# Paleogenomics/pss-bam

Hardware: AMD Instinct MI355X
Metric: aligned reads/s (whole node) + HBM GB/s fraction, 200M x 150bp BAM (higher is better)
Workload: dtype u64

## Files before the change

pss-bam_amd/csrc/bgzf_api.h:

```cpp
#pragma once

#include "inflate_kernels.h"
#include "inflate_wave.h"

extern "C" int64_t pssbam_bgzf_scan(const void *bytes, uint64_t nbytes, pssbam_bgzf_block *blocks, uint64_t max_blocks,
                                    uint64_t *consumed, uint64_t *inflated_bytes) {
    const uint8_t *p = (const uint8_t *)bytes;
    uint64_t o = 0, n = 0, uoff = 0;
    while (o + 18 <= nbytes && (!blocks || n < max_blocks)) {
        if (p[o] != 0x1f || p[o + 1] != 0x8b || p[o + 2] != 8 || !(p[o + 3] & 4)) { fail(PSSBAM_EFORMAT, "not a BGZF block at offset %llu", (unsigned long long)o); return PSSBAM_EFORMAT; }
        const uint32_t xlen = p[o + 10] | ((uint32_t)p[o + 11] << 8);
        if (o + 12 + xlen > nbytes) break;
        uint32_t bsize = 0;
        bool found = false;
        for (uint32_t x = 0; x + 4 <= xlen;) {
            const uint8_t *sf = p + o + 12 + x;
            const uint32_t slen = sf[2] | ((uint32_t)sf[3] << 8);
            if (sf[0] == 'B' && sf[1] == 'C' && slen == 2 && x + 6 <= xlen) { bsize = (sf[4] | ((uint32_t)sf[5] << 8)) + 1u; found = true; break; }
            x += 4 + slen;
        }
        if (!found || bsize < 12u + xlen + 8u) { fail(PSSBAM_EFORMAT, "BGZF block at offset %llu has no usable BC field", (unsigned long long)o); return PSSBAM_EFORMAT; }
        if (o + bsize > nbytes) break;
        uint32_t crc, isize;
        memcpy(&crc, p + o + bsize - 8, 4);
// ... 557 lines not shown
    (void)hipGetLastError();
    size_t limit = FEED_SLOTS_READY;
    if (const char *v = getenv("PSSBAM_FEED_SLOTS")) limit = std::max<size_t>(2, (size_t)atoi(v));
    if (!feed_engine_ready(e)) {
        if (!e->feed_mem_budget) {
            size_t free_b = 0, total_b = 0;
            if (hipMemGetInfo(&free_b, &total_b) != hipSuccess) free_b = 64ull << 30;
            const uint64_t used = e->feed.size() * feed_slot_bytes(e);
            const uint64_t keep = (24ull << 30) + select_reserve_bytes(e) + dedup_reserve_bytes(e) + coverage_reserve_bytes(e);
            e->feed_mem_budget = used + (free_b > keep ? free_b - keep : 0);
        }
        limit = std::max<size_t>(FEED_SLOTS_READY, (size_t)(e->feed_mem_budget / feed_slot_bytes(e)));
        if (const char *v = getenv("PSSBAM_FEED_MAX_SLOTS")) limit = std::max<size_t>(1, (size_t)atoi(v));
    }
    limit = std::min<size_t>(limit, FEED_SLOTS_MAX);
    if (e->feed.size() < limit || (force && oldest < 0 && e->feed.size() < (size_t)FEED_SLOTS_MAX)) {
        const double t0 = feed_now();
        FeedAcc *s = new FeedAcc();
        e->feed.push_back(s);
        const int rc = feed_prepare(e, *s);
        e->feed_t_alloc += feed_now() - t0;
        if (rc) return rc;
        e->feed_slots_allocated++;
        *out_slot = (int)e->feed.size() - 1;
        return PSSBAM_OK;
    }
    if (oldest >= 0) {
        const double t0 = feed_now();
        HIP_TRY(hipEventSynchronize(e->feed[(size_t)oldest]->consumed));
        e->feed_t_wait_busy += feed_now() - t0;
// ... 3 lines not shown
    }
    return fail(PSSBAM_EBUSY, "all %zu feed slots hold inflated records that wait for set_genome / set_references", e->feed.size());
}

static int feed_launch_tally(pssbam_engine *e, const DeferredTally &d) {
    FeedAcc &s = *e->feed[(size_t)d.slot];
    int rc = launch_tally(e, s.d_out + d.sub_base, d.sub_len, s.d_offs + d.offs_at, d.n_bound, nullptr, 0, s.d_nrecs + d.k, d.sample_off);
    if (rc) return rc;
    if (d.last_of_slot) {
        HIP_TRY(hipEventRecord(s.consumed, e->stream));
        s.held = false;
    }
    return PSSBAM_OK;
}

static int feed_resume(pssbam_engine *e) {
    if (e->deferred.empty() || !feed_engine_ready(e)) return PSSBAM_OK;
    HIP_TRY(hipSetDevice(e->device));
    std::vector<DeferredTally> todo;
    todo.swap(e->deferred);
    for (const DeferredTally &d : todo) {
        const int rc = feed_launch_tally(e, d);
        if (rc) return rc;
        e->feed_deferred_launches++;
    }
    return PSSBAM_OK;
}

static int feed_flush(pssbam_engine *e) {
    if (e->cur_feed < 0) return PSSBAM_OK;
    FeedAcc &s = *e->feed[(size_t)e->cur_feed];
    if (s.blocks.empty()) return PSSBAM_OK;
    int rc;
    const double t_flush0 = feed_now();
    if (e->feed_t_first_flush < 0) e->feed_t_first_flush = t_flush0 - e->feed_t0;
    struct FlushTimer { pssbam_engine *e; double t0; ~FlushTimer() { e->feed_t_flush += feed_now() - t0; } } flush_timer{e, t_flush0};
    const size_t nb = s.blocks.size();
    if (nb > 0xFFFFFFF0ull) return fail(PSSBAM_EINVAL, "too many BGZF blocks in one super-batch");
    if (s.blocks_cap < nb) {
        const size_t want = std::max<size_t>(nb, e->feed_block_target < 0xFFFFFFFFull ? (size_t)e->feed_block_target : 0);
        size_t c[8] = {s.blocks_cap, s.blocks_cap, s.blocks_cap, s.blocks_cap, s.blocks_cap, s.blocks_cap, s.blocks_cap, s.blocks_cap};
        if ((rc = grow((uint8_t **)&s.d_blocks, &c[0], want, sizeof(pssbam::BgzfBlock)))) return rc;
        if ((rc = grow(&s.d_a, &c[1], want))) return rc;
        if ((rc = grow(&s.d_e, &c[2], want))) return rc;
        if ((rc = grow(&s.d_last, &c[3], want))) return rc;
        if ((rc = grow(&s.d_nexta, &c[4], want + 1))) return rc;
        if ((rc = grow(&s.d_n, &c[5], want))) return rc;
        if ((rc = grow(&s.d_counts, &c[6], want))) return rc;
// ... 97 lines not shown
        offs_at += sub_len[k] / 36ull + n + 2ull;
    }
    hipLaunchKernelGGL(pssbam::bgzf_chain_carry_out, dim3(1), dim3(256), 0, e->stream, (const uint8_t *)s.d_out, (const uint64_t *)(s.d_chain + 1), data_end,
                       e->d_carry, (uint64_t)FEED_GAP, e->d_feed_tail, e->d_feed_flags);
    HIP_TRY(hipGetLastError());
    HIP_TRY(hipEventRecord(ev1, e->stream));
    if (!s.inflated) HIP_TRY(hipEventCreateWithFlags(&s.inflated, hipEventDisableTiming));
    HIP_TRY(hipEventRecord(s.inflated, e->stream));
    e->inflate_events.emplace_back(ev0, ev1);
    e->inflated_bytes += data_end - FEED_GAP;
    {
        const uint64_t lanes = (uint64_t)e->n_cu * (uint64_t)pssbam::INF_WAVES_PER_CU * 64ull;
        e->feed_blocks_launched += nb;
        e->feed_lanes_launched += (nb + lanes - 1) / lanes * lanes;
    }
    const bool ready = feed_engine_ready(e);
    for (size_t k = 0; k < s.sub_first.size(); k++) {
        DeferredTally d;
        d.slot = e->cur_feed;
        d.sub_base = sub_base[k];
        d.sub_len = sub_len[k];
        d.offs_at = sub_offs[k];
        d.n_bound = (uint32_t)std::min<uint64_t>((k + 1 < sub_offs.size() ? sub_offs[k + 1] : offs_at) - sub_offs[k], 0xFFFFFFF0ull);
        d.k = (uint32_t)k;
        d.sample_off = k == 0 ? FEED_GAP : 0ull;
        d.last_of_slot = k + 1 == s.sub_first.size();
        s.held = true;
        if (ready) { if ((rc = feed_launch_tally(e, d))) return rc; }
        else e->deferred.push_back(d);
    }
    s.busy = true;
// ... 83 lines not shown
    if (first_record_offset > blocks[0].isize) return fail(PSSBAM_EINVAL, "first_record_offset lies beyond the first block");
    for (uint32_t i = 0; i < n_blocks; i++) {
        const pssbam_bgzf_block &b = blocks[i];
        if (b.isize > 65536u || b.in_len > 65536u) return fail(PSSBAM_EINVAL, "blocks[%u]: a BGZF block holds at most 64 KiB (in_len %u, isize %u)", i, b.in_len, b.isize);
        if (b.in_off > comp_bytes || b.in_len > comp_bytes - b.in_off) return fail(PSSBAM_EINVAL, "blocks[%u]: payload lies outside the %llu-byte chunk", i, (unsigned long long)comp_bytes);
        if (i && (b.in_off < blocks[i - 1].in_off + blocks[i - 1].in_len || b.out_off != blocks[i - 1].out_off + blocks[i - 1].isize))
            return fail(PSSBAM_EINVAL, "blocks[%u]: blocks must be in file order with contiguous out_off", i);
    }
    const bool assembling = e->cur_feed >= 0 && !e->feed[(size_t)e->cur_feed]->blocks.empty();
    if (first_record_offset && !(e->feed_fresh && !assembling))
        return fail(PSSBAM_ESTATE, "first_record_offset only makes sense for the first blocks of a stream (after create / reset)");
    if (first_record_offset) e->feed_skip = first_record_offset;
    if (comp_bytes > e->feed_comp_cap / 2) return fail(PSSBAM_EINVAL, "chunk of %llu compressed bytes is too large", (unsigned long long)comp_bytes);
    HIP_TRY(hipSetDevice(e->device));
    if ((rc = feed_state_init(e))) return rc;
    if (!feed_engine_ready(e)) {
        bool fits = false;
        if (e->cur_feed >= 0) {
            const FeedAcc &cur = *e->feed[(size_t)e->cur_feed];
            const uint64_t used = std::max<uint64_t>(cur.out_used, FEED_GAP);
            fits = cur.blocks.size() + n_blocks < e->feed_block_target && used + out_bytes + 8192 <= FEED_GAP + e->feed_out_target &&
                   cur.comp_used + comp_bytes + 64 <= e->feed_comp_cap;
        }
        if (!fits && e->spare_feed < 0) {
            rc = feed_acquire(e, &e->spare_feed, false);
            if (rc) return rc;
        }
    }
    late_streams(e, false);
    hipStream_t cs = (e->ticket_seq & 1u) && e->copy_stream2 ? e->copy_stream2 : e->copy_stream ? e->copy_stream : e->stream;
// ... 156 lines not shown
```

pss-bam_amd/csrc/engine.hip:

```cpp
#include "../../include/pssbam_hip.h"
#include "../../include/fasta-genome-io.h"

#include <hip/hip_runtime.h>

#include <algorithm>
#include <condition_variable>
#include <cstdarg>
#include <cstdio>
#include <cstdlib>
#include <cstring>
#include <ctime>
#include <map>
#include <string>
#include <thread>
#include <tuple>
#include <type_traits>
#include <unordered_map>
#include <unordered_set>
#include <atomic>
#include <memory>
#include <mutex>
#include <vector>

#include "tally_kernels.h"
#include "select_kernels.h"
#include "end_mask_kernels.h"
#include "dedup_kernels.h"
#include "coverage_kernels.h"
#include "allele_kernels.h"
#include "deflate_kernels.h"

using namespace pssbam;

static thread_local char g_err[512] = "";
static double feed_now() {
    timespec ts;
    clock_gettime(CLOCK_MONOTONIC, &ts);
    return ts.tv_sec + ts.tv_nsec * 1e-9;
}
// ... 81 lines not shown
    int slot;
    uint64_t sub_base, sub_len, offs_at;
    uint32_t n_bound, k;
    uint64_t sample_off;
    bool last_of_slot;
};

namespace {
struct PinEntry { size_t len; int refs; };
std::map<const void *, PinEntry> g_pins;
std::mutex g_pins_mu;
bool pin_acquire(const void *p, size_t len) {
    std::lock_guard<std::mutex> lk(g_pins_mu);
    auto it = g_pins.find(p);
    if (it != g_pins.end()) { it->second.refs++; return true; }
    if (hipHostRegister((void *)p, len, hipHostRegisterPortable) != hipSuccess) { (void)hipGetLastError(); return false; }
    g_pins[p] = PinEntry{len, 1};
    return true;
}
void pin_release(const void *p) {
    std::lock_guard<std::mutex> lk(g_pins_mu);
    auto it = g_pins.find(p);
    if (it == g_pins.end()) return;
    if (--it->second.refs == 0) { (void)hipHostUnregister((void *)p); g_pins.erase(it); }
}
}

enum SelectState { SEL_FREE = 0, SEL_TOTALS, SEL_DATA };
struct SelectBuf {
    uint8_t *d_out = nullptr;
    size_t out_cap = 0;
// ... 12 lines not shown
    std::string up_ctx, down_ctx, rg;
    bool has_rg = false;
    int device = 0;
    int n_cu = 0;
    hipStream_t stream = nullptr, copy_stream = nullptr, copy_stream2 = nullptr;
    hipStream_t inflate_stream[2] = {nullptr, nullptr};
    hipEvent_t feed_base_ev = nullptr;
    hipStream_t genome_stream = nullptr;
    std::thread late_thread;
    std::atomic<int> late_ready{0};
    std::mutex late_mu;
    hipStream_t late_copy1 = nullptr, late_copy2 = nullptr, late_genome = nullptr;
    bool late_adopted = false;
    hipEvent_t genome_ready = nullptr;
    bool genome_wait_pending = false;
    std::vector<const void *> genome_pins;
    std::vector<void *> retired;
    hipEvent_t copied2 = nullptr;
    bool own_stream = false;

    uint8_t *d_genome = nullptr;
    uint32_t *d_genome4 = nullptr;
    uint32_t acgt_ctx = 0;
    uint64_t genome_bytes = 0;
    std::vector<uint64_t> contig_start;
    std::vector<uint32_t> contig_len;
    std::vector<std::string> contig_ids;
    int32_t star_contig = -1;
    uint4 *d_ref_info = nullptr;
    uint4 *h_ref_info = nullptr;
// ... 163 lines not shown
    const char *v = getenv(name);
    return v ? atoi(v) : 0;
}

static void late_streams(pssbam_engine *e, bool wait) {
    std::lock_guard<std::mutex> lk(e->late_mu);
    if (e->late_adopted) return;
    if (!wait && !e->late_ready.load(std::memory_order_acquire)) return;
    if (e->late_thread.joinable()) e->late_thread.join();
    e->copy_stream = e->late_copy1;
    e->copy_stream2 = e->late_copy2;
    e->genome_stream = e->late_genome;
    e->late_adopted = true;
}

extern "C" int pssbam_engine_create(const pssbam_config *cfg, pssbam_engine **out) {
    if (!cfg || !out) return fail(PSSBAM_EINVAL, "null argument");
    *out = nullptr;
    if (cfg->abi_version != PSSBAM_ABI_VERSION)
        return fail(PSSBAM_EINVAL, "abi_version %u != %u", cfg->abi_version, PSSBAM_ABI_VERSION);
    if (!(cfg->tally_mask & (PSSBAM_TALLY_PSS | PSSBAM_TALLY_KMER)) ||
        (cfg->tally_mask & ~(PSSBAM_TALLY_PSS | PSSBAM_TALLY_KMER)))
        return fail(PSSBAM_EINVAL, "tally_mask must be a non-empty subset of PSS|KMER");
    if ((cfg->tally_mask & PSSBAM_TALLY_PSS)) {
        if (cfg->pss.region_len < 0 || cfg->pss.region_len > 1000000)
            return fail(PSSBAM_EINVAL, "region_len %d out of range", cfg->pss.region_len);
        if (!cfg->pss.up_ctx || !cfg->pss.down_ctx) return fail(PSSBAM_EINVAL, "up_ctx/down_ctx must be set");
    }
    if ((cfg->tally_mask & PSSBAM_TALLY_KMER) && (cfg->kmer.klen < 1 || cfg->kmer.klen > PSSBAM_MAX_KLEN))
        return fail(PSSBAM_EINVAL, "klen %d outside the device range 1..%d", cfg->kmer.klen, PSSBAM_MAX_KLEN);
// ... 87 lines not shown
    if (const int g = env_int("PSSBAM_REGION_GRID_SHIFT")) e->region_shift = (uint32_t)std::min(std::max(g, 2), 20);
    if (const int g = env_int("PSSBAM_SITE_GRID_SHIFT")) e->site_shift = (uint32_t)std::min(std::max(g, 2), 20);
    if (getenv("PSSBAM_COMPACT")) e->use_compact = env_int("PSSBAM_COMPACT") != 0;
    if (getenv("PSSBAM_COMPACT_PLAN_ONCE")) e->compact_plan_once = env_int("PSSBAM_COMPACT_PLAN_ONCE") != 0;
    if (tstat)
        fprintf(stderr, "[pssbam] engine on device %d: device properties %.3f, its stream + events %.3f, counters + scratch (first allocations, first "
                        "enqueue) %.3f s\n", dev, tc1 - tc0, tc2 - tc1, feed_now() - tc2);
    *out = guard.release();
    return PSSBAM_OK;
}

extern "C" void pssbam_engine_destroy(pssbam_engine *e) {
    if (!e) return;
    (void)hipSetDevice(e->device);
    late_streams(e, true);
    for (hipStream_t is : e->inflate_stream)
        if (is) (void)hipStreamSynchronize(is);
    if (e->stream) (void)hipStreamSynchronize(e->stream);
    if (e->copy_stream) (void)hipStreamSynchronize(e->copy_stream);
    if (e->copy_stream2) (void)hipStreamSynchronize(e->copy_stream2);
    for (Slot &s : e->slots) {
        if (s.d_recs) (void)hipFree(s.d_recs);
        if (s.d_offs) (void)hipFree(s.d_offs);
        if (s.copied) (void)hipEventDestroy(s.copied);
        if (s.copy_begin) (void)hipEventDestroy(s.copy_begin);
        if (s.consumed) (void)hipEventDestroy(s.consumed);
    }
    if (e->genome_stream) (void)hipStreamSynchronize(e->genome_stream);
    for (const void *p : e->genome_pins) pin_release(p);
    e->genome_pins.clear();
// ... 43 lines not shown
    if (e->d_comp_len) (void)hipFree(e->d_comp_len);
    if (e->d_comp_off) (void)hipFree(e->d_comp_off);
    for (void *q : e->retired) (void)hipFree(q);
    if (e->d_feed_tail) (void)hipFree(e->d_feed_tail);
    for (auto &p : e->feed_copies) (void)hipEventDestroy(p.second);
    for (hipEvent_t ev : e->feed_event_pool) (void)hipEventDestroy(ev);
    if (e->d_feed_flags) (void)hipFree(e->d_feed_flags);
    for (auto &p : e->inflate_events) { (void)hipEventDestroy(p.first); (void)hipEventDestroy(p.second); }
    for (auto &p : e->launch_events) { (void)hipEventDestroy(p.first); (void)hipEventDestroy(p.second); }
    for (hipEvent_t ev : e->event_pool) (void)hipEventDestroy(ev);
    if (e->t_begin) (void)hipEventDestroy(e->t_begin);
    if (e->t_end) (void)hipEventDestroy(e->t_end);
    if (e->d_scratch) (void)hipFree(e->d_scratch);
    if (e->d_genome) (void)hipFree(e->d_genome);
    if (e->d_genome4) (void)hipFree(e->d_genome4);
    if (e->d_ref_info) (void)hipFree(e->d_ref_info);
    if (e->h_ref_info) (void)hipHostFree(e->h_ref_info);
    if (e->d_rg) (void)hipFree(e->d_rg);
    for (void *q : {(void *)e->d_region_info, (void *)e->d_region_grid, (void *)e->d_region_iv})
        if (q) (void)hipFree(q);
    if (e->d_score_w) (void)hipFree(e->d_score_w);
    if (e->d_grp_ids) (void)hipFree(e->d_grp_ids);
    if (e->d_grp_offs) (void)hipFree(e->d_grp_offs);
    if (e->d_grp_hash) (void)hipFree(e->d_grp_hash);
    if (e->d_counters_own) (void)hipFree(e->d_counters_own);
    if (e->own_stream && e->stream) (void)hipStreamDestroy(e->stream);
    if (e->copy_stream) (void)hipStreamDestroy(e->copy_stream);
    if (e->copy_stream2) (void)hipStreamDestroy(e->copy_stream2);
    for (hipStream_t is : e->inflate_stream)
        if (is) (void)hipStreamDestroy(is);
    if (e->feed_base_ev) (void)hipEventDestroy(e->feed_base_ev);
    if (e->genome_stream) (void)hipStreamDestroy(e->genome_stream);
    if (e->genome_ready) (void)hipEventDestroy(e->genome_ready);
    if (e->copied2) (void)hipEventDestroy(e->copied2);
    delete e;
}

extern "C" int pssbam_engine_set_stream(pssbam_engine *e, void *hip_stream) {
    if (!e) return fail(PSSBAM_EINVAL, "null engine");
    HIP_TRY(hipSetDevice(e->device));
    HIP_TRY(hipStreamSynchronize(e->stream));
    if (e->own_stream) HIP_TRY(hipStreamDestroy(e->stream));
    e->stream = (hipStream_t)hip_stream;
    e->own_stream = false;
    return PSSBAM_OK;
}

static constexpr uint64_t CONTIG_ALIGN = 256, CONTIG_PAD = 256;

static hipEvent_t take_event(pssbam_engine *e);
static int feed_resume(pssbam_engine *e);
static int coverage_array(pssbam_engine *e, uint64_t genome_bytes);
static void coverage_contigs(pssbam_engine *e);

static int genome_settle(pssbam_engine *e) {
    if (e->genome_pins.empty()) return PSSBAM_OK;
    HIP_TRY(hipSetDevice(e->device));
    HIP_TRY(hipEventSynchronize(e->genome_ready));
    for (const void *p : e->genome_pins) pin_release(p);
    e->genome_pins.clear();
    return PSSBAM_OK;
}

static int genome_upload(pssbam_engine *e, size_t n, const char *const *ids, const uint8_t *const *seqs, const uint64_t *lens,
                         int seqs_on_device) {
    if (!e || (n && (!ids || !seqs || !lens))) return fail(PSSBAM_EINVAL, "null argument");
    HIP_TRY(hipSetDevice(e->device));
    int rc = genome_settle(e);
    if (rc) return rc;
    std::vector<size_t> order(n);
    for (size_t i = 0; i < n; i++) order[i] = i;
    std::stable_sort(order.begin(), order.end(), [&](size_t a, size_t b) { return strcmp(ids[a], ids[b]) < 0; });
    std::vector<uint64_t> start(n + 1, 0);
    std::vector<uint32_t> len(n + 1, 0);
    uint64_t total = CONTIG_PAD;
    for (size_t k = 0; k < n; k++) {
        if (lens[order[k]] > 0xFFFFFF00ull)
            return fail(PSSBAM_EINVAL, "contig %s has %llu bases; the engine addresses contigs below 4 Gi bases", ids[order[k]],
                        (unsigned long long)lens[order[k]]);
        start[k] = total;
        len[k] = (uint32_t)lens[order[k]];
        total += ((uint64_t)len[k] + CONTIG_PAD + CONTIG_ALIGN - 1) / CONTIG_ALIGN * CONTIG_ALIGN;
    }
    if (e->coverage)
        if ((rc = coverage_array(e, total))) return rc;
    if (e->d_genome) {
        HIP_TRY(hipStreamSynchronize(e->stream));
        HIP_TRY(hipFree(e->d_genome));
        e->d_genome = nullptr;
        if (e->d_genome4) { HIP_TRY(hipFree(e->d_genome4)); e->d_genome4 = nullptr; }
    }
    HIP_TRY(hipMalloc(&e->d_genome, total));
    late_streams(e, true);
    if (!e->genome_stream) HIP_TRY(hipStreamCreateWithFlags(&e->genome_stream, hipStreamNonBlocking));
    hipStream_t gs = e->genome_stream;
    if (seqs_on_device) {
        hipEvent_t ev = take_event(e);
        if (!ev) return fail(PSSBAM_EHIP, "hipEventCreate failed");
        HIP_TRY(hipEventRecord(ev, e->stream));
        HIP_TRY(hipStreamWaitEvent(gs, ev, 0));
        e->event_pool.push_back(ev);
    }
    HIP_TRY(hipMemsetAsync(e->d_genome, 0, total, gs));
    const bool try_lock = !seqs_on_device && !getenv("PSSBAM_NO_PIN");
    for (size_t k = 0; k < n; k++) {
        if (!len[k]) continue;
        const void *src = seqs[order[k]];
        if (try_lock && len[k] >= (32u << 20) && pin_acquire(src, len[k])) e->genome_pins.push_back(src);
        HIP_TRY(hipMemcpyAsync(e->d_genome + start[k], src, len[k],
                               seqs_on_device ? hipMemcpyDeviceToDevice : hipMemcpyHostToDevice, gs));
    }
    hipLaunchKernelGGL(encode_genome_kernel, dim3(4096), dim3(256), 0, gs, e->d_genome, total / 16);
    HIP_TRY(hipGetLastError());
    {
        CtxSets sets;
        ctx_mask(e->up_ctx.c_str(), sets.up);
        ctx_mask(e->down_ctx.c_str(), sets.down);
        e->acgt_ctx = 0;
        for (uint32_t v = 0; v < 4; v++)
            e->acgt_ctx |= (((sets.up[0] >> v) & 1u) << (2 * v)) | (((sets.down[0] >> v) & 1u) << (2 * v + 1));
        const uint64_t n_out = total / 8, slack = 16;
        HIP_TRY(hipMalloc(&e->d_genome4, (n_out + slack) * sizeof(uint32_t)));
        HIP_TRY(hipMemsetAsync(e->d_genome4 + n_out, 0x44, slack * sizeof(uint32_t), gs));
        hipLaunchKernelGGL(pack_genome4_kernel, dim3(4096), dim3(256), 0, gs, e->d_genome, e->d_genome4, n_out, sets);
        HIP_TRY(hipGetLastError());
    }
    if (e->coverage) HIP_TRY(hipMemsetAsync(e->d_cov, 0, e->cov_len * sizeof(uint32_t), gs));
    e->site_counts_void = true;
    HIP_TRY(hipEventRecord(e->genome_ready, gs));
    e->genome_wait_pending = true;
    e->contig_start.assign(start.begin(), start.begin() + n);
    e->contig_len.assign(len.begin(), len.begin() + n);
    e->genome_bytes = total;
    e->contig_ids.clear();
    for (size_t k = 0; k < n; k++) e->contig_ids.emplace_back(ids[order[k]]);
    e->star_contig = -1;
    if (e->have_refs) e->have_refs = false;
    {
        auto it = std::lower_bound(e->contig_ids.begin(), e->contig_ids.end(), std::string("*"),
                                   [](const std::string &a, const std::string &b) { return strcmp(a.c_str(), b.c_str()) < 0; });
        if (it != e->contig_ids.end() && *it == "*") e->star_contig = (int32_t)(it - e->contig_ids.begin());
    }
    return PSSBAM_OK;
}

// ... 42 lines not shown
        const uint4 ri = e->ref_info_host[i];
        if (!ri.w) continue;
        const auto it = e->regions.find(i < (size_t)e->n_ref ? e->ref_names[i] : std::string("*"));
        if (it == e->regions.end()) continue;
        uint64_t cnt = 0;
        for (const uint2 &v : it->second) cnt += v.x < ri.z ? 1u : 0u;
        if (!cnt) continue;
        src[i] = &it->second;
        desc[i] = make_uint4(0, (uint32_t)cnt, 0, 0);
        n_iv += cnt;
        n_grid += ((uint64_t)ri.z >> g) + 2;
    }
    if (n_iv >= (1ull << 32) || n_grid >= (1ull << 32)) return fail(PSSBAM_ENOMEM, "the region table has too many intervals or grid words for 32-bit indices");
    const uint64_t bytes = n_ent * sizeof(uint4) + (n_iv + 1) * sizeof(uint2) + (n_grid + 2) * sizeof(uint32_t);
    HIP_TRY(hipSetDevice(e->device));
    if (in_use && e->d_region_info) HIP_TRY(hipStreamSynchronize(e->stream));
    for (void **q : {(void **)&e->d_region_info, (void **)&e->d_region_grid, (void **)&e->d_region_iv})
        if (*q) { HIP_TRY(hipFree(*q)); *q = nullptr; }
    size_t free_b = 0, total_b = 0;
    HIP_TRY(hipMemGetInfo(&free_b, &total_b));
    if (bytes > (uint64_t)free_b)
        return fail(PSSBAM_ENOMEM, "the region table (%llu intervals, grid shift %u) needs %llu bytes; the device has %llu free",
                    (unsigned long long)n_iv, g, (unsigned long long)bytes, (unsigned long long)free_b);
    std::vector<uint2> iv((size_t)n_iv + 1, make_uint2(0, 0));
    std::vector<uint32_t> grid((size_t)n_grid + 2, 0u);
    uint64_t at_iv = 0, at_grid = 0;
    for (size_t i = 0; i < n_ent; i++) {
        if (!src[i]) continue;
        const uint32_t len = e->ref_info_host[i].z, cnt = desc[i].y;
        desc[i].x = (uint32_t)at_iv;
        desc[i].z = (uint32_t)at_grid;
// ... 37 lines not shown
    }
    for (auto &kv : map) {
        std::vector<uint2> &v = kv.second;
        std::sort(v.begin(), v.end(), [](const uint2 &a, const uint2 &b) { return a.x != b.x ? a.x < b.x : a.y < b.y; });
        size_t n = 0;
        for (const uint2 &r : v) {
            if (n && r.x <= v[n - 1].y) v[n - 1].y = std::max(v[n - 1].y, r.y);
            else v[n++] = r;
        }
        v.resize(n);
    }
    HIP_TRY(hipSetDevice(e->device));
    e->regions.swap(map);
    e->has_regions = n_regions > 0;
    if (!e->has_regions) {
        if (e->d_region_info) HIP_TRY(hipStreamSynchronize(e->stream));
        for (void **q : {(void **)&e->d_region_info, (void **)&e->d_region_grid, (void **)&e->d_region_iv})
            if (*q) { HIP_TRY(hipFree(*q)); *q = nullptr; }
        return PSSBAM_OK;
    }
    return e->have_refs ? pack_regions(e, true) : PSSBAM_OK;
}

static void free_sites(pssbam_engine *e) {
    for (void **q : {(void **)&e->d_site_idx, (void **)&e->d_site_grid, (void **)&e->d_site_counts, (void **)&e->d_site_base})
        if (*q) { (void)hipFree(*q); *q = nullptr; }
    e->site_cells = 0;
}

static int pack_sites(pssbam_engine *e) {
    if (!e->has_sites) return PSSBAM_OK;
    HIP_TRY(hipSetDevice(e->device));
    std::vector<uint32_t> old_counts;
    std::vector<uint64_t> old_idx;
    if (e->d_site_idx) {
        HIP_TRY(hipStreamSynchronize(e->stream));
        if (e->tallied && !e->site_counts_void && !e->site_idx.empty()) {
            old_counts.resize(e->site_idx.size() * ALLELE_WORDS);
            HIP_TRY(hipMemcpy(old_counts.data(), e->d_site_counts, old_counts.size() * sizeof(uint32_t), hipMemcpyDeviceToHost));
            old_idx.swap(e->site_idx);
        }
        free_sites(e);
    }
    e->site_counts_void = false;
    e->site_idx.clear();
    e->site_ref.clear();
    e->site_pos.clear();
    e->site_slot.clear();
    std::unordered_set<uint64_t> seen;
    for (size_t i = 0; i < (size_t)e->n_ref; i++) {
        const uint4 ri = e->ref_info_host[i];
// ... 74 lines not shown
        map[names[name_of[i]]].push_back(pos0[i]);
    }
    uint64_t given = 0;
    for (auto &kv : map) {
        std::vector<uint32_t> &v = kv.second;
        std::sort(v.begin(), v.end());
        v.erase(std::unique(v.begin(), v.end()), v.end());
        given += v.size();
    }
    HIP_TRY(hipSetDevice(e->device));
    e->sites.swap(map);
    e->has_sites = n_sites > 0;
    e->site_trim = trim;
    e->sites_given = given;
    if (!e->has_sites) {
        if (e->d_site_idx) HIP_TRY(hipStreamSynchronize(e->stream));
        free_sites(e);
        e->site_idx.clear();
        e->site_ref.clear();
        e->site_pos.clear();
        e->site_slot.clear();
        return PSSBAM_OK;
    }
    return e->have_refs ? pack_sites(e) : PSSBAM_OK;
}

static int size_per_contig(pssbam_engine *e, int32_t n_ref);

extern "C" int pssbam_engine_set_references(pssbam_engine *e, int32_t n_ref, const char *const *names) {
    if (!e || n_ref < 0 || (n_ref && !names)) return fail(PSSBAM_EINVAL, "bad argument");
    if (!e->d_genome) return fail(PSSBAM_ESTATE, "set_genome must precede set_references");
// ... 13 lines not shown
        size_t lo = 0, hi = e->contig_ids.size();
        while (lo < hi) {
            const size_t mid = (lo + hi) / 2;
            const int c = strcmp(names[i], e->contig_ids[mid].c_str());
            if (c == 0) { fill((size_t)i, (int32_t)mid, names[i]); break; }
            if (c < 0) hi = mid; else lo = mid + 1;
        }
    }
    fill((size_t)n_ref, e->star_contig, "*");
    if (e->feed_opened && !e->deferred.empty() && n_ref != e->feed_n_ref)
        return fail(PSSBAM_ESTATE, "pssbam_engine_feed_open announced %d references, set_references brings %d", e->feed_n_ref, n_ref);
    if (e->per_contig)
        if (const int rc = size_per_contig(e, n_ref)) return rc;
    e->ref_names.assign(names, names + n_ref);
    if (e->d_ref_info) {
        if (e->have_refs) HIP_TRY(hipStreamSynchronize(e->stream));
        HIP_TRY(hipFree(e->d_ref_info));
        e->d_ref_info = nullptr;
    }
    HIP_TRY(hipMalloc(&e->d_ref_info, ((size_t)n_ref + 1) * sizeof(uint4)));
    if (e->h_ref_cap < (size_t)n_ref + 1) {
        if (e->h_ref_info) (void)hipHostFree(e->h_ref_info);
        e->h_ref_info = nullptr;
        e->h_ref_cap = (size_t)n_ref + 1 + 64;
        HIP_TRY(hipHostMalloc((void **)&e->h_ref_info, e->h_ref_cap * sizeof(uint4), hipHostMallocDefault));
    } else if (e->have_refs) HIP_TRY(hipStreamSynchronize(e->stream));
    memcpy(e->h_ref_info, info.data(), ((size_t)n_ref + 1) * sizeof(uint4));
    hipLaunchKernelGGL(copy_table_kernel, dim3(1), dim3(256), 0, e->stream, e->d_ref_info, (const uint4 *)e->h_ref_info, (uint32_t)n_ref + 1u);
    HIP_TRY(hipGetLastError());
    const bool replaced = e->have_refs;
    e->n_ref = n_ref;
    e->have_refs = true;
    e->ref_info_host.swap(info);
    coverage_contigs(e);
    if (const int rc = pack_regions(e, replaced)) return rc;
    if (const int rc = pack_sites(e)) return rc;
    return feed_resume(e);
}

static hipEvent_t take_event(pssbam_engine *e) {
    if (!e->event_pool.empty()) {
// ... 844 lines not shown
    rc = resolve_launch_events(e);
    if (rc) return rc;
    if (h2d_ms) *h2d_ms = e->h2d_ms;
    if (h2d_bytes) *h2d_bytes = e->h2d_bytes;
    if (kernel_ms) *kernel_ms = e->kernel_ms;
    if (n_launches) *n_launches = e->kernel_launches;
    return PSSBAM_OK;
}

static int feed_flush(pssbam_engine *e);

extern "C" int pssbam_engine_sync(pssbam_engine *e) {
    if (!e) return fail(PSSBAM_EINVAL, "null engine");
    HIP_TRY(hipSetDevice(e->device));
    {
        const int rc = feed_flush(e);
        if (rc) return rc;
    }
    if (e->copy_stream2) HIP_TRY(hipStreamSynchronize(e->copy_stream2));
    if (e->copy_stream) HIP_TRY(hipStreamSynchronize(e->copy_stream));
    if (e->genome_stream) HIP_TRY(hipStreamSynchronize(e->genome_stream));
    for (hipStream_t q : e->inflate_stream)
        if (q) HIP_TRY(hipStreamSynchronize(q));
    HIP_TRY(hipStreamSynchronize(e->stream));
    const int rc = genome_settle(e);
    if (rc) return rc;
    if (!e->sel_queue.empty())
        if (const int rs = select_poll(e, true)) return rs;
    if (const int rs = select_report(e)) return rs;
    if (!e->deferred.empty())
        return fail(PSSBAM_ESTATE, "compressed blocks were fed (pssbam_engine_feed_open) but set_genome / set_references never followed");
// ... 604 lines not shown
    const size_t tab = (size_t)e->rows * 16;
    if (fwd) memset(fwd, 0, (size_t)n * tab * sizeof(unsigned long));
    if (rev) memset(rev, 0, (size_t)n * tab * sizeof(unsigned long));
    if (touched) memset(touched, 0, (size_t)n);
    return for_touched_planes(e, (uint32_t)first_ref, (uint32_t)n, [&](uint32_t plane, const unsigned long long *p) {
        const size_t i = plane - (uint32_t)first_ref;
        if (touched) touched[i] = 1;
        if (fwd) for (size_t k = 0; k < tab; k++) fwd[i * tab + k] = (unsigned long)p[k];
        if (rev) for (size_t k = 0; k < tab; k++) rev[i * tab + k] = (unsigned long)p[tab + k];
    });
}

extern "C" int pssbam_engine_reset(pssbam_engine *e) {
    if (!e) return fail(PSSBAM_EINVAL, "null engine");
    HIP_TRY(hipSetDevice(e->device));
    if (!e->sel_queue.empty())
        if (const int rs = select_poll(e, true)) return rs;
    if (const int rs = select_report(e)) return rs;
    e->tallied = false;
    e->feed_fresh = true;
    e->feed_skip = 0;
    if (!e->deferred.empty()) {
        e->deferred.clear();
        for (FeedAcc *sp : e->feed)
            if (sp->held) {
                sp->held = false;
                if (!sp->consumed) HIP_TRY(hipEventCreateWithFlags(&sp->consumed, hipEventDisableTiming));
                HIP_TRY(hipEventRecord(sp->consumed, e->stream));
            }
    }
// ... 597 lines not shown
```

pss-bam_amd/csrc/tally_kernels.h:

```cpp
#pragma once

#include "record_decode.h"

namespace pssbam {

constexpr int TILED_THREADS = 256;
constexpr int TILED_WAVES = TILED_THREADS / 64;
constexpr int TILED_ROWS = 32;
constexpr int KMER_LDS_MAX_K = 4;
constexpr uint32_t STAGE_SLACK = 64;
constexpr uint32_t CODE_NONE = 32;
constexpr uint32_t TABLE_WORDS = 64 * 32;
constexpr uint32_t SCRATCH_KMER = 1024, SCRATCH_DELTA = 1536, SCRATCH_WORDS = 1552;
constexpr uint32_t SITE_WORDS = 16 * 32, SITE_SCRATCH_WORDS = SCRATCH_WORDS + SITE_WORDS;
constexpr uint32_t CODE_SITE = 64;
constexpr uint32_t END_SCRATCH_WORDS = SCRATCH_WORDS + 32 * 32;
constexpr uint32_t CODE_END = 64;
__host__ __device__ inline uint32_t end_lds_bytes(uint32_t rows) { return (32u * rows + 4u) * 4u; }
constexpr uint32_t REF_LDS_ENTRIES = 64;

struct LdsTableRowMajor {
    uint32_t *t;
    uint32_t rows;
    __device__ __forceinline__ void add(uint32_t table, uint32_t row, uint32_t cell) const {
// ... 2163 lines not shown
            }
        }
    }
    __syncthreads();
    for (uint32_t i = threadIdx.x; i < n_bins; i += blockDim.x) {
        uint32_t sum = 0u;
        for (uint32_t r = 0; r < rep; r++) sum += lds_hist[(i << rep_log2) + r];
        if (sum) atomicAdd(&bins[bin_lo + i], (unsigned long long)sum);
    }
}

__global__ void copy_table_kernel(uint4 *dst, const uint4 *src, uint32_t n) {
    for (uint32_t i = threadIdx.x; i < n; i += blockDim.x) dst[i] = src[i];
}

__global__ void encode_genome_kernel(uint8_t *p, uint64_t n16) {
    const uint64_t stride = (uint64_t)gridDim.x * blockDim.x;
    uint4 *q = (uint4 *)p;
    for (uint64_t i = (uint64_t)blockIdx.x * blockDim.x + threadIdx.x; i < n16; i += stride) {
        uint4 v = q[i];
        uint32_t w[4] = {v.x, v.y, v.z, v.w};
#pragma unroll
        for (int k = 0; k < 4; k++) {
            uint32_t o = 0;
#pragma unroll
            for (int b = 0; b < 4; b++) {
                uint32_t c = (w[k] >> (8 * b)) & 0xFFu;
                if (c >= 'a' && c <= 'z') c -= 32u;
                o |= enc_byte(c) << (8 * b);
            }
            w[k] = o;
        }
        q[i] = make_uint4(w[0], w[1], w[2], w[3]);
    }
}

struct CtxSets { uint32_t up[8], down[8]; };
__global__ void pack_genome4_kernel(const uint8_t *g, uint32_t *out, uint64_t n_out, CtxSets sets) {
    const uint64_t stride = (uint64_t)gridDim.x * blockDim.x;
    const uint2 *src = (const uint2 *)g;
    for (uint64_t i = (uint64_t)blockIdx.x * blockDim.x + threadIdx.x; i < n_out; i += stride) {
        const uint2 v = src[i];
        uint32_t o = 0u;
#pragma unroll
        for (int b = 0; b < 8; b++) {
            const uint32_t c = ((b < 4 ? v.x : v.y) >> (8 * (b & 3))) & 0xFFu;
            const uint32_t nib = c < 4u ? c : 4u + (in_set(sets.up, c) ? 1u : 0u) + (in_set(sets.down, c) ? 2u : 0u);
            o |= nib << (4 * b);
        }
        out[i] = o;
    }
}

}
```

Before: 23.77 billion.

## Fuse genome encode and nibble packing into one ingest kernel reading host memory directly

Replaces the separate memset, host-to-device copy, encode and pack kernels with a single genome_ingest kernel. The kernel reads contig bytes either from mapped pinned host memory or from a small rotating device staging buffer, and writes both the encoded genome and its 4-bit packed form in one pass. Deferred tally launches now wait until the genome upload event has completed, and are flushed at sync points. This is meant to cut extra HBM passes and copy/memset traffic during genome setup and to overlap BAM inflation with the genome upload. In exchange, zero-copy reads over the host link can be slow, and the deferral adds extra ordering logic.

Result: no change. 23.77 billion (-0.0%).

```diff
diff --git a/pss-bam_amd/csrc/bgzf_api.h b/pss-bam_amd/csrc/bgzf_api.h
--- a/pss-bam_amd/csrc/bgzf_api.h
+++ b/pss-bam_amd/csrc/bgzf_api.h
@@ -595,6 +595,14 @@
         if (const char *v = getenv("PSSBAM_FEED_MAX_SLOTS")) limit = std::max<size_t>(1, (size_t)atoi(v));
     }
     limit = std::min<size_t>(limit, FEED_SLOTS_MAX);
+    if (oldest < 0 && feed_engine_ready(e) && !e->deferred.empty() && e->feed.size() >= limit) {
+        if (const int rc = feed_resume(e, true)) return rc;
+        for (size_t i = 0; i < e->feed.size(); i++) {
+            const FeedAcc &s = *e->feed[i];
+            if ((int)i == e->cur_feed || (int)i == e->spare_feed || !s.busy || s.held) continue;
+            if (oldest < 0 || s.flush_seq < e->feed[(size_t)oldest]->flush_seq) oldest = (int)i;
+        }
+    }
     if (e->feed.size() < limit || (force && oldest < 0 && e->feed.size() < (size_t)FEED_SLOTS_MAX)) {
         const double t0 = feed_now();
         FeedAcc *s = new FeedAcc();
@@ -628,9 +636,10 @@
     return PSSBAM_OK;
 }
 
-static int feed_resume(pssbam_engine *e) {
+static int feed_resume(pssbam_engine *e, bool force) {
     if (e->deferred.empty() || !feed_engine_ready(e)) return PSSBAM_OK;
     HIP_TRY(hipSetDevice(e->device));
+    if (!force && !genome_arrived(e)) return PSSBAM_OK;
     std::vector<DeferredTally> todo;
     todo.swap(e->deferred);
     for (const DeferredTally &d : todo) {
@@ -646,6 +655,7 @@
     FeedAcc &s = *e->feed[(size_t)e->cur_feed];
     if (s.blocks.empty()) return PSSBAM_OK;
     int rc;
+    if ((rc = feed_resume(e))) return rc;
     const double t_flush0 = feed_now();
     if (e->feed_t_first_flush < 0) e->feed_t_first_flush = t_flush0 - e->feed_t0;
     struct FlushTimer { pssbam_engine *e; double t0; ~FlushTimer() { e->feed_t_flush += feed_now() - t0; } } flush_timer{e, t_flush0};
@@ -773,7 +783,7 @@
         e->feed_blocks_launched += nb;
         e->feed_lanes_launched += (nb + lanes - 1) / lanes * lanes;
     }
-    const bool ready = feed_engine_ready(e);
+    const bool ready = feed_engine_ready(e) && e->deferred.empty() && genome_arrived(e);
     for (size_t k = 0; k < s.sub_first.size(); k++) {
         DeferredTally d;
         d.slot = e->cur_feed;
@@ -887,6 +897,7 @@
     if (comp_bytes > e->feed_comp_cap / 2) return fail(PSSBAM_EINVAL, "chunk of %llu compressed bytes is too large", (unsigned long long)comp_bytes);
     HIP_TRY(hipSetDevice(e->device));
     if ((rc = feed_state_init(e))) return rc;
+    if ((rc = feed_resume(e))) return rc;
     if (!feed_engine_ready(e)) {
         bool fits = false;
         if (e->cur_feed >= 0) {
diff --git a/pss-bam_amd/csrc/engine.hip b/pss-bam_amd/csrc/engine.hip
--- a/pss-bam_amd/csrc/engine.hip
+++ b/pss-bam_amd/csrc/engine.hip
@@ -23,6 +23,7 @@
 #include <vector>
 
 #include "tally_kernels.h"
+#include "genome_ingest.h"
 #include "select_kernels.h"
 #include "end_mask_kernels.h"
 #include "dedup_kernels.h"
@@ -134,7 +135,7 @@
     std::lock_guard<std::mutex> lk(g_pins_mu);
     auto it = g_pins.find(p);
     if (it != g_pins.end()) { it->second.refs++; return true; }
-    if (hipHostRegister((void *)p, len, hipHostRegisterPortable) != hipSuccess) { (void)hipGetLastError(); return false; }
+    if (hipHostRegister((void *)p, len, hipHostRegisterPortable | hipHostRegisterMapped) != hipSuccess) { (void)hipGetLastError(); return false; }
     g_pins[p] = PinEntry{len, 1};
     return true;
 }
@@ -177,6 +178,8 @@
     bool late_adopted = false;
     hipEvent_t genome_ready = nullptr;
     bool genome_wait_pending = false;
+    bool genome_in_flight = false;
+    uint8_t *d_genome_stage = nullptr;
     std::vector<const void *> genome_pins;
     std::vector<void *> retired;
     hipEvent_t copied2 = nullptr;
@@ -370,6 +373,8 @@
     e->late_adopted = true;
 }
 
+static int feed_resume(pssbam_engine *e, bool force = false);
+
 extern "C" int pssbam_engine_create(const pssbam_config *cfg, pssbam_engine **out) {
     if (!cfg || !out) return fail(PSSBAM_EINVAL, "null argument");
     *out = nullptr;
@@ -487,6 +492,7 @@
     if (!e) return;
     (void)hipSetDevice(e->device);
     late_streams(e, true);
+    (void)feed_resume(e, true);
     for (hipStream_t is : e->inflate_stream)
         if (is) (void)hipStreamSynchronize(is);
     if (e->stream) (void)hipStreamSynchronize(e->stream);
@@ -560,6 +566,7 @@
     if (e->d_scratch) (void)hipFree(e->d_scratch);
     if (e->d_genome) (void)hipFree(e->d_genome);
     if (e->d_genome4) (void)hipFree(e->d_genome4);
+    if (e->d_genome_stage) (void)hipFree(e->d_genome_stage);
     if (e->d_ref_info) (void)hipFree(e->d_ref_info);
     if (e->h_ref_info) (void)hipHostFree(e->h_ref_info);
     if (e->d_rg) (void)hipFree(e->d_rg);
@@ -585,6 +592,7 @@
 extern "C" int pssbam_engine_set_stream(pssbam_engine *e, void *hip_stream) {
     if (!e) return fail(PSSBAM_EINVAL, "null engine");
     HIP_TRY(hipSetDevice(e->device));
+    if (const int rc = feed_resume(e, true)) return rc;
     HIP_TRY(hipStreamSynchronize(e->stream));
     if (e->own_stream) HIP_TRY(hipStreamDestroy(e->stream));
     e->stream = (hipStream_t)hip_stream;
@@ -595,7 +603,11 @@
 static constexpr uint64_t CONTIG_ALIGN = 256, CONTIG_PAD = 256;
 
 static hipEvent_t take_event(pssbam_engine *e);
-static int feed_resume(pssbam_engine *e);
+static int drain_stream(pssbam_engine *e) {
+    if (const int rc = feed_resume(e, true)) return rc;
+    HIP_TRY(hipStreamSynchronize(e->stream));
+    return PSSBAM_OK;
+}
 static int coverage_array(pssbam_engine *e, uint64_t genome_bytes);
 static void coverage_contigs(pssbam_engine *e);
 
@@ -608,6 +620,14 @@
     return PSSBAM_OK;
 }
 
+static bool genome_arrived(pssbam_engine *e) {
+    if (!e->genome_in_flight) return true;
+    if (hipEventQuery(e->genome_ready) == hipSuccess) { e->genome_in_flight = false; return true; }
+    (void)hipGetLastError();
+    return false;
+}
+
+static constexpr uint64_t GENOME_STAGE_BYTES = 32ull << 20;
 static int genome_upload(pssbam_engine *e, size_t n, const char *const *ids, const uint8_t *const *seqs, const uint64_t *lens,
                          int seqs_on_device) {
     if (!e || (n && (!ids || !seqs || !lens))) return fail(PSSBAM_EINVAL, "null argument");
@@ -628,6 +648,7 @@
         len[k] = (uint32_t)lens[order[k]];
         total += ((uint64_t)len[k] + CONTIG_PAD + CONTIG_ALIGN - 1) / CONTIG_ALIGN * CONTIG_ALIGN;
     }
+    if (e->d_genome && (rc = feed_resume(e, true))) return rc;
     if (e->coverage)
         if ((rc = coverage_array(e, total))) return rc;
     if (e->d_genome) {
@@ -636,7 +657,9 @@
         e->d_genome = nullptr;
         if (e->d_genome4) { HIP_TRY(hipFree(e->d_genome4)); e->d_genome4 = nullptr; }
     }
+    const uint64_t n_out = total / 8, slack = 16;
     HIP_TRY(hipMalloc(&e->d_genome, total));
+    HIP_TRY(hipMalloc(&e->d_genome4, (n_out + slack) * sizeof(uint32_t)));
     late_streams(e, true);
     if (!e->genome_stream) HIP_TRY(hipStreamCreateWithFlags(&e->genome_stream, hipStreamNonBlocking));
     hipStream_t gs = e->genome_stream;
@@ -647,34 +670,55 @@
         HIP_TRY(hipStreamWaitEvent(gs, ev, 0));
         e->event_pool.push_back(ev);
     }
-    HIP_TRY(hipMemsetAsync(e->d_genome, 0, total, gs));
+    CtxSets sets;
+    ctx_mask(e->up_ctx.c_str(), sets.up);
+    ctx_mask(e->down_ctx.c_str(), sets.down);
+    e->acgt_ctx = 0;
+    for (uint32_t v = 0; v < 4; v++)
+        e->acgt_ctx |= (((sets.up[0] >> v) & 1u) << (2 * v)) | (((sets.down[0] >> v) & 1u) << (2 * v + 1));
+    HIP_TRY(hipMemsetAsync(e->d_genome4 + n_out, 0x44, slack * sizeof(uint32_t), gs));
+    auto ingest = [&](const uint8_t *src, uint64_t src_len, uint64_t at, uint64_t groups, bool over_link) {
+        const uint64_t grid = std::min<uint64_t>((groups + 255) / 256, (uint64_t)e->n_cu * (over_link ? 1u : 8u));
+        hipLaunchKernelGGL(genome_ingest_kernel, dim3((uint32_t)grid), dim3(256), 0, gs, src, src_len, e->d_genome + at, e->d_genome4 + at / 8, groups,
+                           sets);
+    };
+    ingest(nullptr, 0, 0, CONTIG_PAD / 16, false);
     const bool try_lock = !seqs_on_device && !getenv("PSSBAM_NO_PIN");
+    uint64_t stage_at = 0;
     for (size_t k = 0; k < n; k++) {
-        if (!len[k]) continue;
-        const void *src = seqs[order[k]];
-        if (try_lock && len[k] >= (32u << 20) && pin_acquire(src, len[k])) e->genome_pins.push_back(src);
-        HIP_TRY(hipMemcpyAsync(e->d_genome + start[k], src, len[k],
-                               seqs_on_device ? hipMemcpyDeviceToDevice : hipMemcpyHostToDevice, gs));
-    }
-    hipLaunchKernelGGL(encode_genome_kernel, dim3(4096), dim3(256), 0, gs, e->d_genome, total / 16);
+        const uint8_t *src = seqs[order[k]];
+        const uint64_t region = ((uint64_t)len[k] + CONTIG_PAD + CONTIG_ALIGN - 1) / CONTIG_ALIGN * CONTIG_ALIGN;
+        if (seqs_on_device || !len[k]) {
+            ingest(src, len[k], start[k], region / 16, false);
+            continue;
+        }
+        if (try_lock && len[k] >= (32u << 20) && pin_acquire(src, len[k])) {
+            void *dp = nullptr;
+            if (hipHostGetDevicePointer(&dp, (void *)src, 0) == hipSuccess && dp) {
+                e->genome_pins.push_back(src);
+                ingest((const uint8_t *)dp, len[k], start[k], region / 16, true);
+                continue;
+            }
+            (void)hipGetLastError();
+            pin_release(src);
+        }
+        if (!e->d_genome_stage) HIP_TRY(hipMalloc(&e->d_genome_stage, GENOME_STAGE_BYTES));
+        for (uint64_t done = 0; done < len[k];) {
+            const uint64_t piece = std::min<uint64_t>(len[k] - done, GENOME_STAGE_BYTES);
+            if (stage_at + piece > GENOME_STAGE_BYTES) stage_at = 0;
+            HIP_TRY(hipMemcpyAsync(e->d_genome_stage + stage_at, src + done, piece, hipMemcpyHostToDevice, gs));
+            const bool last = done + piece == len[k];
+            ingest(e->d_genome_stage + stage_at, piece, start[k] + done, last ? (region - done) / 16 : piece / 16, false);
+            stage_at += (piece + 15) & ~15ull;
+            done += piece;
+        }
+    }
     HIP_TRY(hipGetLastError());
-    {
-        CtxSets sets;
-        ctx_mask(e->up_ctx.c_str(), sets.up);
-        ctx_mask(e->down_ctx.c_str(), sets.down);
-        e->acgt_ctx = 0;
-        for (uint32_t v = 0; v < 4; v++)
-            e->acgt_ctx |= (((sets.up[0] >> v) & 1u) << (2 * v)) | (((sets.down[0] >> v) & 1u) << (2 * v + 1));
-        const uint64_t n_out = total / 8, slack = 16;
-        HIP_TRY(hipMalloc(&e->d_genome4, (n_out + slack) * sizeof(uint32_t)));
-        HIP_TRY(hipMemsetAsync(e->d_genome4 + n_out, 0x44, slack * sizeof(uint32_t), gs));
-        hipLaunchKernelGGL(pack_genome4_kernel, dim3(4096), dim3(256), 0, gs, e->d_genome, e->d_genome4, n_out, sets);
-        HIP_TRY(hipGetLastError());
-    }
     if (e->coverage) HIP_TRY(hipMemsetAsync(e->d_cov, 0, e->cov_len * sizeof(uint32_t), gs));
     e->site_counts_void = true;
     HIP_TRY(hipEventRecord(e->genome_ready, gs));
     e->genome_wait_pending = true;
+    e->genome_in_flight = true;
     e->contig_start.assign(start.begin(), start.begin() + n);
     e->contig_len.assign(len.begin(), len.begin() + n);
     e->genome_bytes = total;
@@ -747,7 +791,8 @@
     if (n_iv >= (1ull << 32) || n_grid >= (1ull << 32)) return fail(PSSBAM_ENOMEM, "the region table has too many intervals or grid words for 32-bit indices");
     const uint64_t bytes = n_ent * sizeof(uint4) + (n_iv + 1) * sizeof(uint2) + (n_grid + 2) * sizeof(uint32_t);
     HIP_TRY(hipSetDevice(e->device));
-    if (in_use && e->d_region_info) HIP_TRY(hipStreamSynchronize(e->stream));
+    if (in_use && e->d_region_info)
+        if (const int rc = drain_stream(e)) return rc;
     for (void **q : {(void **)&e->d_region_info, (void **)&e->d_region_grid, (void **)&e->d_region_iv})
         if (*q) { HIP_TRY(hipFree(*q)); *q = nullptr; }
     size_t free_b = 0, total_b = 0;
@@ -815,7 +860,8 @@
     e->regions.swap(map);
     e->has_regions = n_regions > 0;
     if (!e->has_regions) {
-        if (e->d_region_info) HIP_TRY(hipStreamSynchronize(e->stream));
+        if (e->d_region_info)
+            if (const int rc = drain_stream(e)) return rc;
         for (void **q : {(void **)&e->d_region_info, (void **)&e->d_region_grid, (void **)&e->d_region_iv})
             if (*q) { HIP_TRY(hipFree(*q)); *q = nullptr; }
         return PSSBAM_OK;
@@ -835,7 +881,7 @@
     std::vector<uint32_t> old_counts;
     std::vector<uint64_t> old_idx;
     if (e->d_site_idx) {
-        HIP_TRY(hipStreamSynchronize(e->stream));
+        if (const int rc = drain_stream(e)) return rc;
         if (e->tallied && !e->site_counts_void && !e->site_idx.empty()) {
             old_counts.resize(e->site_idx.size() * ALLELE_WORDS);
             HIP_TRY(hipMemcpy(old_counts.data(), e->d_site_counts, old_counts.size() * sizeof(uint32_t), hipMemcpyDeviceToHost));
@@ -940,7 +986,8 @@
     e->site_trim = trim;
     e->sites_given = given;
     if (!e->has_sites) {
-        if (e->d_site_idx) HIP_TRY(hipStreamSynchronize(e->stream));
+        if (e->d_site_idx)
+            if (const int rc = drain_stream(e)) return rc;
         free_sites(e);
         e->site_idx.clear();
         e->site_ref.clear();
@@ -984,7 +1031,8 @@
         if (const int rc = size_per_contig(e, n_ref)) return rc;
     e->ref_names.assign(names, names + n_ref);
     if (e->d_ref_info) {
-        if (e->have_refs) HIP_TRY(hipStreamSynchronize(e->stream));
+        if (e->have_refs)
+            if (const int rc = drain_stream(e)) return rc;
         HIP_TRY(hipFree(e->d_ref_info));
         e->d_ref_info = nullptr;
     }
@@ -994,7 +1042,9 @@
         e->h_ref_info = nullptr;
         e->h_ref_cap = (size_t)n_ref + 1 + 64;
         HIP_TRY(hipHostMalloc((void **)&e->h_ref_info, e->h_ref_cap * sizeof(uint4), hipHostMallocDefault));
-    } else if (e->have_refs) HIP_TRY(hipStreamSynchronize(e->stream));
+    } else if (e->have_refs) {
+        if (const int rc = drain_stream(e)) return rc;
+    }
     memcpy(e->h_ref_info, info.data(), ((size_t)n_ref + 1) * sizeof(uint4));
     hipLaunchKernelGGL(copy_table_kernel, dim3(1), dim3(256), 0, e->stream, e->d_ref_info, (const uint4 *)e->h_ref_info, (uint32_t)n_ref + 1u);
     HIP_TRY(hipGetLastError());
@@ -1869,7 +1919,8 @@
     if (!e) return fail(PSSBAM_EINVAL, "null engine");
     HIP_TRY(hipSetDevice(e->device));
     {
-        const int rc = feed_flush(e);
+        int rc = feed_flush(e);
+        if (!rc) rc = feed_resume(e, true);
         if (rc) return rc;
     }
     if (e->copy_stream2) HIP_TRY(hipStreamSynchronize(e->copy_stream2));
@@ -2504,6 +2555,7 @@
 extern "C" int pssbam_engine_reset(pssbam_engine *e) {
     if (!e) return fail(PSSBAM_EINVAL, "null engine");
     HIP_TRY(hipSetDevice(e->device));
+    if (const int rc = feed_resume(e, true)) return rc;
     if (!e->sel_queue.empty())
         if (const int rs = select_poll(e, true)) return rs;
     if (const int rs = select_report(e)) return rs;
diff --git a/pss-bam_amd/csrc/genome_ingest.h b/pss-bam_amd/csrc/genome_ingest.h
--- /dev/null
+++ b/pss-bam_amd/csrc/genome_ingest.h
@@ -0,0 +1,72 @@
+#pragma once
+#include <hip/hip_runtime.h>
+#include <stdint.h>
+
+#include "record_decode.h"
+
+namespace pssbam {
+
+struct CtxSets { uint32_t up[8], down[8]; };
+
+__global__ void __launch_bounds__(256) genome_ingest_kernel(const uint8_t *__restrict__ src, uint64_t src_len, uint8_t *__restrict__ dst,
+                                                            uint32_t *__restrict__ dst4, uint64_t n_groups, CtxSets sets) {
+    const uint32_t lane = threadIdx.x & 63u;
+    const uint64_t wave = ((uint64_t)blockIdx.x * blockDim.x + threadIdx.x) >> 6;
+    const uint64_t n_waves = ((uint64_t)gridDim.x * blockDim.x) >> 6;
+    const uint32_t a = (uint32_t)((uintptr_t)src & 15u);
+    const uint4 *lines = (const uint4 *)(src - a);
+    for (uint64_t g0 = wave * 64u; g0 < n_groups; g0 += n_waves * 64u) {
+        const uint64_t g = g0 + lane;
+        uint32_t w[4] = {0u, 0u, 0u, 0u};
+        const bool wide = (a == 0u || g0 > 0u) && (g0 + 64u) * 16u + (a ? 16u : 0u) <= src_len;
+        if (wide) {
+            const uint4 v = lines[g];
+            if (a == 0u) {
+                w[0] = v.x; w[1] = v.y; w[2] = v.z; w[3] = v.w;
+            } else {
+                uint4 nx;
+                nx.x = __shfl_down(v.x, 1);
+                nx.y = __shfl_down(v.y, 1);
+                nx.z = __shfl_down(v.z, 1);
+                nx.w = __shfl_down(v.w, 1);
+                if (lane == 63u) nx = lines[g + 1];
+                uint32_t t0, t1, t2, t3, t4;
+                switch (a >> 2) {
+                case 0: t0 = v.x; t1 = v.y; t2 = v.z; t3 = v.w; t4 = nx.x; break;
+                case 1: t0 = v.y; t1 = v.z; t2 = v.w; t3 = nx.x; t4 = nx.y; break;
+                case 2: t0 = v.z; t1 = v.w; t2 = nx.x; t3 = nx.y; t4 = nx.z; break;
+                default: t0 = v.w; t1 = nx.x; t2 = nx.y; t3 = nx.z; t4 = nx.w; break;
+                }
+                const uint32_t sh = (a & 3u) * 8u;
+                w[0] = __funnelshift_r(t0, t1, sh);
+                w[1] = __funnelshift_r(t1, t2, sh);
+                w[2] = __funnelshift_r(t2, t3, sh);
+                w[3] = __funnelshift_r(t3, t4, sh);
+            }
+        } else {
+            if (g >= n_groups) continue;
+            const uint64_t c0 = g * 16u;
+#pragma unroll
+            for (int b = 0; b < 16; b++)
+                if (c0 + (uint64_t)b < src_len) w[b >> 2] |= (uint32_t)src[c0 + (uint64_t)b] << (8 * (b & 3));
+        }
+        uint32_t o[4], nib[2] = {0u, 0u};
+#pragma unroll
+        for (int k = 0; k < 4; k++) {
+            o[k] = 0u;
+#pragma unroll
+            for (int b = 0; b < 4; b++) {
+                uint32_t c = (w[k] >> (8 * b)) & 0xFFu;
+                if (c >= 'a' && c <= 'z') c -= 32u;
+                const uint32_t s = enc_byte(c);
+                o[k] |= s << (8 * b);
+                const uint32_t n = s < 4u ? s : 4u + (in_set(sets.up, s) ? 1u : 0u) + (in_set(sets.down, s) ? 2u : 0u);
+                nib[k >> 1] |= n << (4 * (b + 4 * (k & 1)));
+            }
+        }
+        ((uint4 *)dst)[g] = make_uint4(o[0], o[1], o[2], o[3]);
+        ((uint2 *)dst4)[g] = make_uint2(nib[0], nib[1]);
+    }
+}
+
+}
diff --git a/pss-bam_amd/csrc/tally_kernels.h b/pss-bam_amd/csrc/tally_kernels.h
--- a/pss-bam_amd/csrc/tally_kernels.h
+++ b/pss-bam_amd/csrc/tally_kernels.h
@@ -2201,42 +2201,4 @@
     for (uint32_t i = threadIdx.x; i < n; i += blockDim.x) dst[i] = src[i];
 }
 
-__global__ void encode_genome_kernel(uint8_t *p, uint64_t n16) {
-    const uint64_t stride = (uint64_t)gridDim.x * blockDim.x;
-    uint4 *q = (uint4 *)p;
-    for (uint64_t i = (uint64_t)blockIdx.x * blockDim.x + threadIdx.x; i < n16; i += stride) {
-        uint4 v = q[i];
-        uint32_t w[4] = {v.x, v.y, v.z, v.w};
-#pragma unroll
-        for (int k = 0; k < 4; k++) {
-            uint32_t o = 0;
-#pragma unroll
-            for (int b = 0; b < 4; b++) {
-                uint32_t c = (w[k] >> (8 * b)) & 0xFFu;
-                if (c >= 'a' && c <= 'z') c -= 32u;
-                o |= enc_byte(c) << (8 * b);
-            }
-            w[k] = o;
-        }
-        q[i] = make_uint4(w[0], w[1], w[2], w[3]);
-    }
-}
-
-struct CtxSets { uint32_t up[8], down[8]; };
-__global__ void pack_genome4_kernel(const uint8_t *g, uint32_t *out, uint64_t n_out, CtxSets sets) {
-    const uint64_t stride = (uint64_t)gridDim.x * blockDim.x;
-    const uint2 *src = (const uint2 *)g;
-    for (uint64_t i = (uint64_t)blockIdx.x * blockDim.x + threadIdx.x; i < n_out; i += stride) {
-        const uint2 v = src[i];
-        uint32_t o = 0u;
-#pragma unroll
-        for (int b = 0; b < 8; b++) {
-            const uint32_t c = ((b < 4 ? v.x : v.y) >> (8 * (b & 3))) & 0xFFu;
-            const uint32_t nib = c < 4u ? c : 4u + (in_set(sets.up, c) ? 1u : 0u) + (in_set(sets.down, c) ? 2u : 0u);
-            o |= nib << (4 * b);
-        }
-        out[i] = o;
-    }
-}
-
-}
+}
```
